# boycehbz/MvSMPLfitting

Measured on AMD Instinct MI355X. Metric: L-BFGS closure evaluations per second (fwd+bwd, all concurrently fitted problems), 8-view 1-person 4-stage fits, higher is better.
Workload: dtype f32

## Files before the change

### mvsmplfitting_amd/csrc/closure_device.h

```cpp
#pragma once
#include <cstddef>
#include "mvfit_device.h"

namespace mvfit {

struct ObsBlock {
    float camR[MVFIT_MAX_VIEWS][9];
    float camt[MVFIT_MAX_VIEWS][3];
    float camf[MVFIT_MAX_VIEWS];
    float camc[MVFIT_MAX_VIEWS][2];
    float gt[MVFIT_MAX_VIEWS * NKP * 2];
    float wc[MVFIT_MAX_VIEWS * NKP];
    float gt3d[NKP * 3];
    float c3d[NKP];
};
struct PoseBlock {
    float theta[72];
    float R[NJ][9];
    float rod[NJ][3];
    float J[NJ][3];
    float Mj[32][12];
    float G[NJ][12];
    float A[NJ][12];
};
// ... 492 lines not shown
            L.pose.Mj[j][4 * (e / 3) + (e % 3)] = (j == 0 ? L.opt.x[X_SC] : 1.0f) * sel;
            if (e < 3) L.pose.rod[j][e] = rod[e];
        } else {
            const int a = e - 9;
            const int pa = L.M.parents[j];
            float s = L.M.J_t[3 * j + a];
#pragma unroll
            for (int l = 0; l < 10; ++l) s = fmaf(L.M.J_S[3 * j + a][l], L.opt.x[X_BETAS + l], s);
            float sp = 0.f;
            if (j > 0) {
                sp = L.M.J_t[3 * pa + a];
#pragma unroll
                for (int l = 0; l < 10; ++l) sp = fmaf(L.M.J_S[3 * pa + a][l], L.opt.x[X_BETAS + l], sp);
            }
            L.pose.J[j][a] = s;
            L.pose.Mj[j][4 * a + 3] = s - sp;
        }
    }
    __syncthreads();
}

template <bool REMOTE = false>
__device__ __attribute__((noinline)) void pose_prep_decode(const DevModel& M, ClosureLds& L, uint32_t flags, int tid) {
    pose_prep_decode_inl<REMOTE>(M, L, flags, tid);
}

template <bool CALL = false>
__device__ __forceinline__ void pose_prep(const DevModel& M, ClosureLds& L, uint32_t flags, int tid) {
    if constexpr (CALL) pose_prep_decode<false>(M, L, flags, tid);
    else pose_prep_decode_inl<false>(M, L, flags, tid);
    pose_prep_elems(M, L, flags, tid);
}

__device__ __forceinline__ void chain_forward_wave(ClosureLds& L, int lane) {
    if (lane < 12) L.pose.G[0][lane] = L.pose.Mj[0][lane];
    const int q = lane / 12, e = lane - 12 * q, a = e >> 2, c = e & 3;
    const int npass = L.M.n_fwd;
    constexpr int CH = 8;
    wave_lds_fence();
    for (int p0 = 0; p0 < npass; p0 += CH) {
        int w[CH];
        float m0[CH], m1[CH], m2[CH];
#pragma unroll
        for (int u = 0; u < CH; ++u) w[u] = (q < 5 && p0 + u < npass) ? L.M.fwd_tab[p0 + u][q] : -1;
#pragma unroll
        for (int u = 0; u < CH; ++u) {
            const int j = w[u] >= 0 ? (w[u] & 0xff) : 0;
            m0[u] = L.pose.Mj[j][c]; m1[u] = L.pose.Mj[j][4 + c]; m2[u] = L.pose.Mj[j][8 + c];
        }
#pragma unroll
        for (int u = 0; u < CH; ++u) {
            if (p0 + u < npass) {
                if (w[u] >= 0) {
                    const int j = w[u] & 0xff, pa = w[u] >> 8;
                    const float4 g = *reinterpret_cast<const float4*>(&L.pose.G[pa][4 * a]);
                    float v = g.x * m0[u] + g.y * m1[u] + g.z * m2[u];
                    if (c == 3) v += g.w;
                    L.pose.G[j][e] = v;
                }
                wave_lds_fence();
            }
        }
    }
    for (int i = lane; i < NJ * 3; i += 64) {
        const int j = i / 3, aa = i - 3 * j;
        const float4 g = *reinterpret_cast<const float4*>(&L.pose.G[j][4 * aa]);
        const float t = g.w - (g.x * L.pose.J[j][0] + g.y * L.pose.J[j][1] + g.z * L.pose.J[j][2]);
        *reinterpret_cast<float4*>(&L.pose.A[j][4 * aa]) = make_float4(g.x, g.y, g.z, t);
    }
}

__device__ __forceinline__ void chain_forward_block(ClosureLds& L, int tid) {
    const bool act = tid < NJ * 12;
    const int j = act ? tid / 12 : 0, e = tid - 12 * j, a = e >> 2, c = e & 3;
    const int ns = L.M.n_jump;
    int anc[5];
#pragma unroll
    for (int s = 0; s < 5; ++s) anc[s] = L.M.anc_tab[s][j];
    const float* src = &L.pose.Mj[0][0];
    float* dst = &L.pose.G[0][0];
#pragma unroll
    for (int s = 0; s < 5; ++s) {
        if (s < ns) {
            if (act) {
                float v;
                if (anc[s] >= 0) {
                    const float4 x = *reinterpret_cast<const float4*>(src + anc[s] * 12 + 4 * a);
                    v = x.x * src[j * 12 + c] + x.y * src[j * 12 + 4 + c] + x.z * src[j * 12 + 8 + c];
                    if (c == 3) v += x.w;
                } else {
                    v = src[j * 12 + e];
                }
                dst[j * 12 + e] = v;
            }
            __syncthreads();
            src = dst;
// ... 303 lines not shown
            const float* mu = M.gmm_means + m * 69;
            float qd = 0.f;
            for (int r = l16; r < 69; r += 16) qd = fmaf(L.gmm_t[m][r], L.pose.theta[3 + r] - mu[r], qd);
            qd = row16_sum(qd);
            if (l16 == 0) L.gmm_ll[m] = 0.5f * qd - M.gmm_lognw[m];
        }
    }
    __syncthreads();
    double total = 0.0;
    if constexpr (!DEFER) total = loss_combine<false>(M, L, V, W, tid == 0);
    const bool use_3d = (W.flags & MVFIT_F_USE_3D) != 0;
    if (want_grad && tid < 3) {
        float s = 0.f;
        for (int w = 0; w < ndw; ++w) s += L.red_f[w][tid];
        if (use_3d) for (int k = 0; k < NKP; ++k) s += L.gkp3[k][tid];
        L.gtau[tid] = s;
    }
    if (want_grad && tid >= 64 && tid < 64 + NKP * 3) {
        const int i = tid - 64;
        float s = 0.f;
#pragma unroll
        for (int vv = 0; vv < MVFIT_MAX_VIEWS; ++vv) if (vv < V) s += (&L.gkp_part[vv][0][0])[i];
        if (use_3d) s += (&L.gkp3[0][0])[i];
        (&L.gkp[0][0])[i] = s;
    }
    return total;
}

__device__ __forceinline__ void chain_backward_wave(ClosureLds& L, int lane) {
    const int q = lane / 12, e = lane - 12 * q, a = e >> 2, m = e & 3;
    const int mr = m < 3 ? m : 0;
    const int npass = L.M.n_bwd;
    constexpr int CH = 4;
    wave_lds_fence();
    for (int p0 = 0; p0 < npass; p0 += CH) {
        int w[CH];
        float4 k0[CH], k1[CH], k2[CH];
        float own[CH];
#pragma unroll
        for (int u = 0; u < CH; ++u) w[u] = (q < 5 && p0 + u < npass) ? L.M.bwd_tab[p0 + u][q] : -1;
#pragma unroll
        for (int u = 0; u < CH; ++u) {
            const int ww = w[u] != -1 ? w[u] : 0x1f1f1f00;
            const int c0 = (ww >> 8) & 0xff, c1 = (ww >> 16) & 0xff, c2 = (ww >> 24) & 0xff;
            k0[u] = *reinterpret_cast<const float4*>(&L.pose.Mj[c0][4 * mr]);
            k1[u] = *reinterpret_cast<const float4*>(&L.pose.Mj[c1][4 * mr]);
            k2[u] = *reinterpret_cast<const float4*>(&L.pose.Mj[c2][4 * mr]);
            own[u] = L.gG[ww & 0x1f][e];
        }
#pragma unroll
        for (int u = 0; u < CH; ++u) {
            if (p0 + u < npass) {
                if (w[u] != -1) {
                    const int p = w[u] & 0x1f, c0 = (w[u] >> 8) & 0xff, c1 = (w[u] >> 16) & 0xff, c2 = (w[u] >> 24) & 0xff;
                    const float4 g0 = *reinterpret_cast<const float4*>(&L.gG[c0][4 * a]);
                    const float4 g1 = *reinterpret_cast<const float4*>(&L.gG[c1][4 * a]);
                    const float4 g2 = *reinterpret_cast<const float4*>(&L.gG[c2][4 * a]);
                    float acc;
                    if (m < 3) {
                        acc = (g0.x * k0[u].x + g0.y * k0[u].y + g0.z * k0[u].z + g0.w * k0[u].w) +
                              (g1.x * k1[u].x + g1.y * k1[u].y + g1.z * k1[u].z + g1.w * k1[u].w) +
                              (g2.x * k2[u].x + g2.y * k2[u].y + g2.z * k2[u].z + g2.w * k2[u].w);
                    } else {
                        acc = g0.w + g1.w + g2.w;
                    }
                    const float base = (w[u] & 0x80) ? L.gG[p][e] : own[u];
                    L.gG[p][e] = base + acc;
                }
                wave_lds_fence();
            }
        }
    }
}

constexpr int BWD_SLICES = 8, BWD_CPS = NC_MAX / BWD_SLICES;
__device__ __forceinline__ int bwd_slices(int) { return BWD_SLICES; }

template <int CPS>
__device__ __forceinline__ void contraction_backward_t(const DevModel& M, ClosureLds& L, int t, int nthreads) {
    constexpr int npq = KROWS >> 2;
    const int nc_pad = L.M.nc_pad;
    const int cps = ((nc_pad >> 2) + BWD_SLICES - 1) / BWD_SLICES * 4;
    for (int item = t; item < npq * BWD_SLICES; item += nthreads) {
        const int pq = item % npq, cs = (item / npq + (int)blockIdx.x) & (BWD_SLICES - 1);
        const int c0 = cs * cps;
        const float4* src = reinterpret_cast<const float4*>(M.pd_subT) + pq;
        float4 v[CPS];
#pragma unroll
        for (int r = 0; r < CPS; ++r) {
            const int c = min(c0 + r, nc_pad - 1);
            if (CPS == BWD_CPS ? r < cps : true) v[r] = src[(size_t)c * npq];
        }
        float4 acc0 = make_float4(0.f, 0.f, 0.f, 0.f), acc1 = acc0;
#pragma unroll
        for (int r = 0; r < CPS; r += 2) {
            if (r < cps) {
                const float g0 = L.gvp[c0 + r], g1 = L.gvp[c0 + r + 1];
                acc0.x = fmaf(g0, v[r].x, acc0.x); acc0.y = fmaf(g0, v[r].y, acc0.y);
                acc0.z = fmaf(g0, v[r].z, acc0.z); acc0.w = fmaf(g0, v[r].w, acc0.w);
                acc1.x = fmaf(g1, v[r + 1].x, acc1.x); acc1.y = fmaf(g1, v[r + 1].y, acc1.y);
                acc1.z = fmaf(g1, v[r + 1].z, acc1.z); acc1.w = fmaf(g1, v[r + 1].w, acc1.w);
            }
        }
        float4* dst = reinterpret_cast<float4*>(L.scratch + cs * KROWS + 4 * pq);
        *dst = make_float4(acc0.x + acc1.x, acc0.y + acc1.y, acc0.z + acc1.z, acc0.w + acc1.w);
    }
}

__device__ __forceinline__ void contraction_backward(const DevModel& M, ClosureLds& L, int t, int nthreads) {
    constexpr int SMPL_CPS = 28;
    if (((L.M.nc_pad >> 2) + BWD_SLICES - 1) / BWD_SLICES * 4 <= SMPL_CPS) contraction_backward_t<SMPL_CPS>(M, L, t, nthreads);
    else contraction_backward_t<BWD_CPS>(M, L, t, nthreads);
}

template <bool REMOTE = false, bool DEFER = false, bool SDFW = false>
__device__ __forceinline__ void closure_backward(const DevModel& M, ClosureLds& L, int V, const DevWeights& W, int tid) {
    const bool use_vp = (W.flags & MVFIT_F_VPOSER) != 0;
    const int ns = L.M.ns, nc = L.M.nc, nc_pad = L.M.nc_pad;
    __syncthreads();
    if constexpr (DEFER) {
        static_assert(NC_MAX + NJ * 3 <= STEP_NT - 64, "E5's threads leave the last wave free");
        if (tid >= STEP_NT - 64) loss_combine<SDFW>(M, L, V, W, tid == STEP_NT - 64);
    }
    if (tid < nc_pad) {
        float v = 0.f;
        if (tid < nc) {
            const int s = tid / 3, bq = tid - 3 * s;
            float gx0 = 0.f, gx1 = 0.f, gx2 = 0.f;
            if (L.M.padded) {
#pragma unroll
                for (int t = 0; t < VS_NZ; ++t) {
                    const int k = L.M.vsp_k[s][t];
                    const float w = L.M.vsp_w[s][t];
                    gx0 = fmaf(w, L.gkp[k][0], gx0); gx1 = fmaf(w, L.gkp[k][1], gx1); gx2 = fmaf(w, L.gkp[k][2], gx2);
                }
            } else {
                for (int t = L.M.vs_start[s]; t < L.M.vs_start[s + 1]; ++t) {
                    const int k = L.M.vs_k[t];
                    const float w = L.M.vs_w[t];
                    gx0 = fmaf(w, L.gkp[k][0], gx0); gx1 = fmaf(w, L.gkp[k][1], gx1); gx2 = fmaf(w, L.gkp[k][2], gx2);
                }
            }
            v = L.T[s][0 + bq] * gx0 + L.T[s][4 + bq] * gx1 + L.T[s][8 + bq] * gx2;
            L.gx[tid] = bq == 0 ? gx0 : (bq == 1 ? gx1 : gx2);
        }
        L.gvp[tid] = v;
    } else if (tid < NC_MAX) {
        L.gvp[tid] = 0.f;
    } else if (tid < NC_MAX + NJ * 3 && L.M.n_skel) {
        const int i = tid - NC_MAX, j = i / 3, a = i - 3 * j;
        float gs = 0.f;
        for (int k = 0; k < NKP; ++k) if (kp_joint_of(L.M, k) == j) gs += L.gkp[k][a];
        L.gM[j][a] = gs;
    }
    __syncthreads();
    PH_T(4);
    const float sdf_fac = L.sdf_fac;
    if (tid < NJ * 16) {
        const int j = tid >> 4, g = tid & 15;
        float acc[12];
#pragma unroll
        for (int e = 0; e < 12; ++e) acc[e] = 0.f;
        for (int s = g; s < ns; s += 16) {
            const float w = L.M.wT[j][s];
            const float g0 = w * L.gx[3 * s], g1 = w * L.gx[3 * s + 1], g2 = w * L.gx[3 * s + 2];
            const float v0 = L.vposed[3 * s], v1 = L.vposed[3 * s + 1], v2 = L.vposed[3 * s + 2];
            acc[0] = fmaf(g0, v0, acc[0]); acc[1] = fmaf(g0, v1, acc[1]); acc[2] = fmaf(g0, v2, acc[2]);
            acc[3] = fmaf(g1, v0, acc[3]); acc[4] = fmaf(g1, v1, acc[4]); acc[5] = fmaf(g1, v2, acc[5]);
            acc[6] = fmaf(g2, v0, acc[6]); acc[7] = fmaf(g2, v1, acc[7]); acc[8] = fmaf(g2, v2, acc[8]);
            acc[9] += g0; acc[10] += g1; acc[11] += g2;
        }
#pragma unroll
        for (int e = 0; e < 12; ++e) acc[e] = row16_sum(acc[e]);
        if (g == 0) {
            if (sdf_fac != 0.f) {
#pragma unroll
                for (int e = 0; e < 12; ++e) acc[e] = fmaf(sdf_fac, sdf_ld(&L.sdf_adj->gA[j * 12 + e]), acc[e]);
            }
            const float J0 = L.pose.J[j][0], J1 = L.pose.J[j][1], J2 = L.pose.J[j][2];
#pragma unroll
            for (int a = 0; a < 3; ++a) {
                *reinterpret_cast<float4*>(&L.gG[j][4 * a]) =
                    make_float4(acc[3 * a + 0] - acc[9 + a] * J0, acc[3 * a + 1] - acc[9 + a] * J1,
                                acc[3 * a + 2] - acc[9 + a] * J2, L.M.n_skel ? acc[9 + a] + L.gM[j][a] : acc[9 + a]);
                L.gJ[j][a] = -(L.pose.G[j][0 + a] * acc[9] + L.pose.G[j][4 + a] * acc[10] + L.pose.G[j][8 + a] * acc[11]);
            }
        }
    }
    __syncthreads();
    PH_T(5);
    const long long t_e7 = PH_CLK();
    if (tid < 64) { chain_backward_wave(L, tid); PH_T(23); }
    else { contraction_backward(M, L, tid - 64, STEP_NT - 64); PH_W(59, 64, t_e7); PH_W(61, 448, t_e7); }
    const int ncs = bwd_slices(STEP_NT - 64);
    __syncthreads();
    PH_T(6);
    auto gm_elem = [&](int pa, int j, int mm, int c) -> float {
        float v = L.pose.G[pa][mm] * L.gG[j][c] + L.pose.G[pa][4 + mm] * L.gG[j][4 + c] + L.pose.G[pa][8 + mm] * L.gG[j][8 + c];
        asm volatile("" : "+v"(v));
        return v;
    };
    constexpr int GJ_T0 = 320;
    static_assert(GJ_T0 >= NJ * 12 && GJ_T0 % 64 == 0 && GJ_T0 + NJ * 3 <= STEP_NT, "g_J totals on otherwise idle waves");
    if (tid >= GJ_T0 && tid < GJ_T0 + NJ * 3) {
        const int i = tid - GJ_T0, j = i / 3, a = i - 3 * j;
        const int c_lo = L.M.child_start[j], c_hi = L.M.child_start[j + 1];
        int ch[3];
#pragma unroll
        for (int k = 0; k < 3; ++k) ch[k] = c_lo + k < c_hi ? L.M.child_list[min(c_lo + k, NJ - 1)] : NJ;
        float gj = L.gJ[j][a] + (j == 0 ? L.gG[0][4 * a + 3] : gm_elem(L.M.parents[j], j, a, 3));
        float sub[3];
#pragma unroll
        for (int k = 0; k < 3; ++k) sub[k] = gm_elem(j, ch[k], a, 3);
#pragma unroll
        for (int k = 0; k < 3; ++k) gj -= sub[k];
        for (int ci = c_lo + 3; ci < c_hi; ++ci) gj -= gm_elem(j, L.M.child_list[ci], a, 3);
        L.gvp[i] = gj;
    }
    if (tid < NJ * 12) {
        const int j = tid / 12, e = tid - 12 * j, mm = e >> 2, c = e & 3;
        float v;
        if (j == 0) v = L.gG[0][e];
        else {
            const int pa = L.M.parents[j];
            v = L.pose.G[pa][mm] * L.gG[j][c] + L.pose.G[pa][4 + mm] * L.gG[j][4 + c] + L.pose.G[pa][8 + mm] * L.gG[j][8 + c];
        }
        L.gM[j][e] = v;
// ... 228 lines not shown
```

### mvsmplfitting_amd/csrc/model_layout.h

```cpp
#pragma once
#include <stdint.h>

namespace mvfit {

constexpr int NJ = 24;
constexpr int NKP = 17;
constexpr int KROWS = 224;
constexpr int KGROUPS = 28;
constexpr int TILE_V = 32;
constexpr int NS_MAX = 96;
constexpr int NS_STRIDE = 112;
constexpr int NC_MAX = NS_MAX * 3;
constexpr int KNNZ_MAX = 160;
constexpr int KP_NZ = 12;
constexpr int VS_NZ = 2;
constexpr int VPS_SLICES = 8;

struct ModelLds {
    float wT[NJ][NS_STRIDE];
    float J_t[NJ * 3];
    float J_S[NJ * 3][11];
    float vt_sub[NC_MAX];
    int sel_v[NS_MAX];
    int kp_start[NKP + 1];
    int kp_s[KNNZ_MAX];
    float kp_w[KNNZ_MAX];
    int vs_start[NS_MAX + 1];
    int vs_k[KNNZ_MAX];
    float vs_w[KNNZ_MAX];
    int kpp_s[NKP][KP_NZ];
    float kpp_w[NKP][KP_NZ];
    int vsp_k[NS_MAX][VS_NZ];
    float vsp_w[NS_MAX][VS_NZ];
    int padded;
    unsigned kp_joint[3];
    int parents[NJ];
    int nlevels;
    int level_start[NJ + 1];
    int level_joints[NJ];
    int child_start[NJ + 1];
    int child_list[NJ];
    int n_fwd, n_bwd;
    int fwd_tab[NJ][5];
    int bwd_tab[NJ][5];
    int anc_tab[5][NJ];
    int n_jump, n_skel, jpad1, jpad2;
    int ns, nc, nc_pad, pad0;
    float selw[NS_MAX][4];
    unsigned selj[NS_MAX];
    int sel_sparse, spad0, spad1, spad2;
};
static_assert(sizeof(ModelLds) % 16 == 0, "ModelLds is bulk-copied as 16-byte words");
static_assert(NKP <= 18 && NJ < 31, "kp_joint packs six 5-bit entries per word");

}
```

### mvsmplfitting_amd/csrc/model_prep.cpp

```cpp
#include "model_prep.h"

#include <math.h>
#include <algorithm>
#include <cmath>
#include <cstdarg>
#include <cstdio>
#include <cstring>

namespace mvfit {
namespace {

constexpr int NPOSE = 207;
constexpr int NBASIS = 217;

int fail(std::string& err, int code, const char* fmt, ...) {
    char buf[512];
    va_list ap;
    va_start(ap, fmt);
    vsnprintf(buf, sizeof(buf), fmt, ap);
    va_end(ap);
    err = buf;
    return code;
}

// ... 165 lines not shown
    for (int s = 0; s < ns; ++s) {
        G.vs_start[s] = nnz;
        for (int k = 0; k < NKP; ++k) {
            const double w = ksel[(size_t)k * nv + sel[s]];
            if (w == 0.0) continue;
            G.vs_k[nnz] = k; G.vs_w[nnz] = (float)w; ++nnz;
        }
    }
    for (int s = ns; s <= NS_MAX; ++s) G.vs_start[s] = nnz;
    G.padded = 1;
    for (int k = 0; k < NKP; ++k) {
        const int n0 = G.kp_start[k], cnt = G.kp_start[k + 1] - n0;
        if (cnt > KP_NZ) G.padded = 0;
        for (int t = 0; t < KP_NZ; ++t) { G.kpp_s[k][t] = t < cnt ? G.kp_s[n0 + t] : 0; G.kpp_w[k][t] = t < cnt ? G.kp_w[n0 + t] : 0.f; }
    }
    for (int s = 0; s < NS_MAX; ++s) {
        const int n0 = G.vs_start[s], cnt = G.vs_start[s + 1] - n0;
        if (cnt > VS_NZ) G.padded = 0;
        for (int t = 0; t < VS_NZ; ++t) { G.vsp_k[s][t] = t < cnt ? G.vs_k[n0 + t] : 0; G.vsp_w[s][t] = t < cnt ? G.vs_w[n0 + t] : 0.f; }
    }
    h.tile_sel_start.assign(h.ntiles + 1, 0);
    h.tile_sel_local.assign(ns, 0);
    h.tile_sel_slot.assign(ns, 0);
    int pos = 0;
    for (int T = 0; T < h.ntiles; ++T) {
        h.tile_sel_start[T] = pos;
        for (int s = 0; s < ns; ++s)
            if (sel[s] / TILE_V == T) { h.tile_sel_local[pos] = sel[s] % TILE_V; h.tile_sel_slot[pos] = s; ++pos; }
    }
    h.tile_sel_start[h.ntiles] = pos;
    return MVFIT_OK;
}

int build_chain(const mvfit_model& m, ModelLds& G, std::string& err) {
    int depth[NJ];
    for (int j = 0; j < NJ; ++j) {
        G.parents[j] = m.parents[j];
        if (j > 0 && (m.parents[j] < 0 || m.parents[j] >= j)) return fail(err, MVFIT_E_ARG, "parents must be topologically ordered");
        depth[j] = j == 0 ? 0 : depth[m.parents[j]] + 1;
    }
    int maxd = 0;
    for (int j = 0; j < NJ; ++j) maxd = std::max(maxd, depth[j]);
    G.nlevels = maxd + 1;
    int pos = 0;
    for (int lv = 0; lv <= maxd; ++lv) {
        G.level_start[lv] = pos;
        for (int j = 0; j < NJ; ++j) if (depth[j] == lv) G.level_joints[pos++] = j;
    }
    for (int lv = maxd + 1; lv <= NJ; ++lv) G.level_start[lv] = pos;
    pos = 0;
    for (int p = 0; p < NJ; ++p) {
        G.child_start[p] = pos;
        for (int j = 1; j < NJ; ++j) if (m.parents[j] == p) G.child_list[pos++] = j;
    }
    G.child_start[NJ] = pos;
    memset(G.fwd_tab, 0xff, sizeof(G.fwd_tab));
    memset(G.bwd_tab, 0xff, sizeof(G.bwd_tab));
    int np = 0;
    for (int lv = 1; lv <= maxd; ++lv)
        for (int base = G.level_start[lv]; base < G.level_start[lv + 1]; base += 5, ++np) {
            if (np >= NJ) return fail(err, MVFIT_E_UNSUPPORTED, "kinematic tree needs more than %d chain passes", NJ);
            for (int q = 0; q < 5 && base + q < G.level_start[lv + 1]; ++q) {
                const int j = G.level_joints[base + q];
                G.fwd_tab[np][q] = j | (m.parents[j] << 8);
            }
        }
// ... 11 lines not shown
    np = 0;
    for (int lv = maxd - 1; lv >= 0; --lv) {
        std::vector<int> entries;
        for (int i = G.level_start[lv]; i < G.level_start[lv + 1]; ++i) {
            const int p = G.level_joints[i];
            const int nc = G.child_start[p + 1] - G.child_start[p];
            for (int k = 0; k < nc; k += 3) {
                int ch[3] = {31, 31, 31};
                for (int t = 0; t < 3 && k + t < nc; ++t) ch[t] = G.child_list[G.child_start[p] + k + t];
                entries.push_back(p | (k > 0 ? 0x80 : 0) | (ch[0] << 8) | (ch[1] << 16) | (ch[2] << 24));
            }
        }
        std::vector<bool> used(entries.size(), false);
        size_t left = entries.size();
        while (left > 0) {
            if (np >= NJ) return fail(err, MVFIT_E_UNSUPPORTED, "kinematic tree needs more than %d adjoint passes", NJ);
            int q = 0;
            std::vector<int> parents_in_pass;
            for (size_t i = 0; i < entries.size() && q < 5; ++i) {
                if (used[i]) continue;
                const int p = entries[i] & 0x1f;
                bool clash = false;
                for (int pp : parents_in_pass) clash |= pp == p;
                if (clash) continue;
                G.bwd_tab[np][q++] = entries[i];
                parents_in_pass.push_back(p);
                used[i] = true;
                --left;
            }
            ++np;
        }
    }
    G.n_bwd = np;
    return MVFIT_OK;
}

int build_vposer(const mvfit_model& m, HostModel& h, std::string& err) {
    if (!m.vp_fc1_w) return MVFIT_OK;
    if (!m.vp_fc1_b || !m.vp_fc2_w || !m.vp_fc2_b || !m.vp_out_w || !m.vp_out_b) return fail(err, MVFIT_E_ARG, "incomplete vposer weights");
    const std::vector<float>&w1 = h.vp_w1, &w2 = h.vp_w2, &w3 = h.vp_w3;
    h.vp_w1.assign(m.vp_fc1_w, m.vp_fc1_w + 512 * 32); h.vp_b1.assign(m.vp_fc1_b, m.vp_fc1_b + 512);
    h.vp_w2.assign(m.vp_fc2_w, m.vp_fc2_w + 512 * 512); h.vp_b2.assign(m.vp_fc2_b, m.vp_fc2_b + 512);
    h.vp_w3.assign(m.vp_out_w, m.vp_out_w + 138 * 512); h.vp_b3.assign(m.vp_out_b, m.vp_out_b + 138);
    h.vp_w1T.assign(32 * 512, 0.f); h.vp_w2T.assign(512 * 512, 0.f); h.vp_w3T.assign(512 * 144, 0.f);
    for (int o = 0; o < 512; ++o) for (int i = 0; i < 32; ++i) h.vp_w1T[i * 512 + o] = w1[o * 32 + i];
    for (int o = 0; o < 512; ++o) for (int i = 0; i < 512; ++i) h.vp_w2T[i * 512 + o] = w2[o * 512 + i];
    for (int o = 0; o < 138; ++o) for (int i = 0; i < 512; ++i) h.vp_w3T[i * 144 + o] = w3[o * 512 + i];
    h.vp_tw2.assign((size_t)VPS_SLICES * 16 * 512 * 4, 0.f);
    h.vp_tw3.assign((size_t)VPS_SLICES * 6 * 512 * 4, 0.f);
    for (int hs = 0; hs < VPS_SLICES; ++hs)
        for (int tid = 0; tid < 512; ++tid) {
            const int w = tid >> 6, l = tid & 63;
            for (int j = 0; j < 16; ++j)
                for (int q = 0; q < 4; ++q)
                    h.vp_tw2[(((size_t)hs * 16 + j) * 512 + tid) * 4 + q] = w2[(size_t)(64 * hs + 8 * w + (j >> 1)) * 512 + 8 * l + 4 * (j & 1) + q];
            for (int j = 0; j < 6; ++j) {
                const int o = l + 64 * (j >> 1);
                if (o < 138)
                    for (int q = 0; q < 4; ++q)
                        h.vp_tw3[(((size_t)hs * 6 + j) * 512 + tid) * 4 + q] = w3[(size_t)o * 512 + 64 * hs + 8 * w + 4 * (j & 1) + q];
            }
        }
    h.has_vposer = true;
    return MVFIT_OK;
}

// ... 58 lines not shown
```

### mvsmplfitting_amd/csrc/mvfit_api.hip

```cpp
#include <dlfcn.h>
#include <hip/hip_runtime.h>

#include <algorithm>
#include <cmath>
#include <cstdarg>
#include <cstdio>
#include <cstdlib>
#include <cstring>
#include <string>
#include <vector>

#include "closure_device.h"
#include "model_prep.h"

namespace mvfit {

hipError_t launch_vertex_pass(const DevModel& M, const DevPose& P, int B, float* verts, int ksplit,
                              hipStream_t stream, hipEvent_t ev_start = nullptr, hipEvent_t ev_stop = nullptr);
hipError_t vertex_pass_configure();
hipError_t launch_pass_gate(const DevPose& P, int b_lo, int B, hipStream_t stream);
hipError_t launch_vertex_pass_resident(const DevModel& M, const ResidentArgs& RA, int tpw, hipStream_t stream);
hipError_t launch_sdf_term(const DevModel& M, const DevPose& P, const float* verts, int B, const int32_t* faces, int num_faces,
                           int G, const int* gate, SdfBox* box, float4* samp, void* entries, SdfAdj* adj, hipStream_t stream,
                           void* cull, unsigned* answer_tag = nullptr, unsigned answer = 0u, const unsigned long long* box_parts = nullptr);
// ... 261 lines not shown
        for (int e = 0; e < LB_EPL; ++e) {
            const int i = LB_EPL * tid + e;
            gnew[e] = i < D ? L.grad[cmap(i, use_vp)] : 0.f;
        }
    }
    lbfgs_round<float, STEP_NT, REUSE>(&L.opt.lbS, &L.opt.lbV[0], H, L.lbW, O, (double)(float)total, gnew, xt, tid, stage_final, [&]() {
        PH_T(10);
        if constexpr (COMPACT) lb_direction_compact<float, STEP_NT>(H, L.lbW, tid);
        else lb_direction_block<float, STEP_NT>(H, L.lbW, tid, GL);
        PH_T(11); PH_ADD(15, 1);
    });
    if (tid < 64) {
#pragma unroll
        for (int e = 0; e < LB_EPL; ++e) {
            const int i = LB_EPL * tid + e;
            if (i < D) L.opt.x[cmap(i, use_vp)] = xt[e];
        }
        if (tid == 0) { L.sh_stage = min(L.opt.lbS.stage, O.num_stages - 1); L.sh_status = L.opt.lbS.status; }
        PH_ADD(13, 1); PH_ADD(14, L.opt.lbS.hist_len);
    }
    __syncthreads();
    PH_T(12);
    return L.sh_status != 0;
}

constexpr int kHistLdFull = 88, kHistLdVp = 52;
__host__ __device__ constexpr int persistent_hist_ld(bool vp) { return vp ? kHistLdVp : kHistLdFull; }
__host__ __device__ constexpr size_t persistent_tail_offset(bool vp) {
    return vp ? ((sizeof(ClosureLds) + 15) & ~(size_t)15) : offsetof(ClosureLds, vp_pre1);
}
__host__ __device__ constexpr size_t persistent_lds_bytes(bool vp) {
    return persistent_tail_offset(vp) + ((size_t)2 * LB_HIST * persistent_hist_ld(vp) + LB_RPACK) * sizeof(float);
}
static_assert(persistent_lds_bytes(false) <= 160 * 1024 && persistent_lds_bytes(true) <= 160 * 1024, "one workgroup per CU: 160 KB of LDS");

__device__ __forceinline__ size_t step_lds_dev() { return (sizeof(ClosureLds) + 15) & ~(size_t)15; }

template <bool REUSE>
__global__ __launch_bounds__(STEP_NT) void fit_step_kernel(DevModel M, const ObsBlock* __restrict__ obs, int nviews,
                                                           StageWeights SW, LbOpts O, DevPose P, FitBuffers F) {
    extern __shared__ __attribute__((aligned(16))) unsigned char smem_raw[];
    ClosureLds& L = *reinterpret_cast<ClosureLds*>(smem_raw);
    const int b = blockIdx.x, tid = threadIdx.x;
    PH_T0();
    prologue(L, M, obs + b, F.pose + b, F.opt + b, P.vposed_sel + (size_t)b * NC_MAX, P.xs_sel + (size_t)b * NC_MAX, nullptr, tid,
             F.sdf_adj ? F.sdf_adj + b : nullptr, (SW.w[0].flags & MVFIT_F_VPOSER) ? F.vp + b : nullptr);
    opts_in(L, SW, O, tid);
    __syncthreads();
    if (L.opt.lbS.status != 0) return;
    if (tid == 0) { L.sh_stage = L.opt.lbS.stage; L.sh_status = 0; }
    LbHist<float> H{F.dirs + (size_t)b * LB_HIST * LB_D, F.stps + (size_t)b * LB_HIST * LB_D, L.opt.lb_ro,
                    F.grow + (size_t)b * LB_GSIZE, F.gcol + (size_t)b * LB_GSIZE};
    __syncthreads();
    float warm = 0.f;
    {
        const int n0 = L.opt.lbS.hist_len, head0 = L.opt.lbS.hist_head;
        constexpr int LPR = LB_D * 4 / 128;
        if (tid < 2 * LPR * n0) {
            const int which = tid / (LPR * n0), r = tid - which * LPR * n0, age = r / LPR, ln = r - age * LPR;
            int slot = head0 + age;
            slot = slot >= LB_HIST ? slot - LB_HIST : slot;
            warm = (which ? H.stps : H.dirs)[slot * LB_D + ln * 32];
        }
    }
    LbGramLds GL{reinterpret_cast<float*>(smem_raw + step_lds_dev()), L.opt.lbS.hist_head,
                 min(L.opt.lbS.hist_len + 1, LB_HIST) + 3 + 4 * LB_PD};
    lb_gram_dma<STEP_NT>(H.gcol, GL.row0, GL.buf, GL.nrows, tid);
// ... 1823 lines not shown
```

Baseline: 1.544 million.

## Pass kinematic chain values through lane shuffles and rebalance backward contraction across waves

```diff
diff --git a/mvsmplfitting_amd/csrc/closure_device.h b/mvsmplfitting_amd/csrc/closure_device.h
--- a/mvsmplfitting_amd/csrc/closure_device.h
+++ b/mvsmplfitting_amd/csrc/closure_device.h
@@ -548,17 +548,48 @@
     pose_prep_elems(M, L, flags, tid);
 }
 
+template <int SEL>
+__device__ __forceinline__ float quad_bcast(float v) { return dpp_mov<SEL * 0x55>(v); }
+__device__ __forceinline__ float lane_fetch(float v, int src_lane) {
+    return __builtin_bit_cast(float, __builtin_amdgcn_ds_bpermute(src_lane << 2, __builtin_bit_cast(int, v)));
+}
+__device__ __forceinline__ float4 quad_row(float t) {
+    return make_float4(quad_bcast<0>(t), quad_bcast<1>(t), quad_bcast<2>(t), quad_bcast<3>(t));
+}
+
+__device__ __forceinline__ float chain_fwd_elem(const float4& g, float m0, float m1, float m2, bool last_col) {
+#pragma clang fp contract(off)
+    const float p1 = g.y * m1, p2 = g.z * m2;
+    float v = fmaf(g.x, m0, p1) + p2;
+    if (last_col) v += g.w;
+    return v;
+}
+__device__ __forceinline__ float chain_bwd_elem(const float4& g0, const float4& g1, const float4& g2, const float4& k0,
+                                                const float4& k1, const float4& k2, bool rot) {
+#pragma clang fp contract(off)
+    if (!rot) return g0.w + g1.w + g2.w;
+    const float a0 = ((g0.x * k0.x + g0.y * k0.y) + g0.z * k0.z) + g0.w * k0.w;
+    const float a1 = fmaf(g1.w, k1.w, fmaf(g1.z, k1.z, fmaf(g1.y, k1.y, g1.x * k1.x)));
+    const float a2 = fmaf(g2.w, k2.w, fmaf(g2.z, k2.z, fmaf(g2.y, k2.y, g2.x * k2.x)));
+    return (a0 + a1) + a2;
+}
+
 __device__ __forceinline__ void chain_forward_wave(ClosureLds& L, int lane) {
-    if (lane < 12) L.pose.G[0][lane] = L.pose.Mj[0][lane];
     const int q = lane / 12, e = lane - 12 * q, a = e >> 2, c = e & 3;
+    float cur = lane < 12 ? L.pose.Mj[0][lane] : 0.f;
+    if (lane < 12) L.pose.G[0][lane] = cur;
     const int npass = L.M.n_fwd;
     constexpr int CH = 8;
-    wave_lds_fence();
     for (int p0 = 0; p0 < npass; p0 += CH) {
-        int w[CH];
+        int w[CH], src[CH], fb[CH];
         float m0[CH], m1[CH], m2[CH];
 #pragma unroll
-        for (int u = 0; u < CH; ++u) w[u] = (q < 5 && p0 + u < npass) ? L.M.fwd_tab[p0 + u][q] : -1;
+        for (int u = 0; u < CH; ++u) {
+            const bool in = q < 5 && p0 + u < npass;
+            w[u] = in ? L.M.fwd_tab[p0 + u][q] : -1;
+            src[u] = in ? (int)L.M.fwd_src[p0 + u][q] : 0xff;
+            fb[u] = p0 + u < npass ? (int)L.M.fwd_src[p0 + u][5] : 0;
+        }
 #pragma unroll
         for (int u = 0; u < CH; ++u) {
             const int j = w[u] >= 0 ? (w[u] & 0xff) : 0;
@@ -567,17 +598,20 @@
 #pragma unroll
         for (int u = 0; u < CH; ++u) {
             if (p0 + u < npass) {
+                float4 g = quad_row(lane_fetch(cur, 12 * (src[u] & 7) + e));
+                const bool lds = wave_uniform(fb[u]) != 0;
+                if (lds) wave_lds_fence();
                 if (w[u] >= 0) {
                     const int j = w[u] & 0xff, pa = w[u] >> 8;
-                    const float4 g = *reinterpret_cast<const float4*>(&L.pose.G[pa][4 * a]);
-                    float v = g.x * m0[u] + g.y * m1[u] + g.z * m2[u];
-                    if (c == 3) v += g.w;
+                    if (lds && src[u] == 0xff) g = *reinterpret_cast<const float4*>(&L.pose.G[pa][4 * a]);
+                    const float v = chain_fwd_elem(g, m0[u], m1[u], m2[u], c == 3);
                     L.pose.G[j][e] = v;
+                    cur = v;
                 }
-                wave_lds_fence();
-            }
-        }
-    }
+            }
+        }
+    }
+    wave_lds_fence();
     for (int i = lane; i < NJ * 3; i += 64) {
         const int j = i / 3, aa = i - 3 * j;
         const float4 g = *reinterpret_cast<const float4*>(&L.pose.G[j][4 * aa]);
@@ -947,13 +981,19 @@
     const int mr = m < 3 ? m : 0;
     const int npass = L.M.n_bwd;
     constexpr int CH = 4;
+    float cur = 0.f;
     wave_lds_fence();
     for (int p0 = 0; p0 < npass; p0 += CH) {
-        int w[CH];
-        float4 k0[CH], k1[CH], k2[CH];
+        int w[CH], src[CH], fb[CH];
+        float4 k0[CH], k1[CH], k2[CH], s0[CH], s1[CH], s2[CH];
         float own[CH];
 #pragma unroll
-        for (int u = 0; u < CH; ++u) w[u] = (q < 5 && p0 + u < npass) ? L.M.bwd_tab[p0 + u][q] : -1;
+        for (int u = 0; u < CH; ++u) {
+            const bool in = q < 5 && p0 + u < npass;
+            w[u] = in ? L.M.bwd_tab[p0 + u][q] : -1;
+            src[u] = in ? (int)L.M.bwd_src[p0 + u][q] : 0;
+            fb[u] = p0 + u < npass ? (int)L.M.fwd_src[p0 + u][6] : 0;
+        }
 #pragma unroll
         for (int u = 0; u < CH; ++u) {
             const int ww = w[u] != -1 ? w[u] : 0x1f1f1f00;
@@ -962,152 +1002,202 @@
             k1[u] = *reinterpret_cast<const float4*>(&L.pose.Mj[c1][4 * mr]);
             k2[u] = *reinterpret_cast<const float4*>(&L.pose.Mj[c2][4 * mr]);
             own[u] = L.gG[ww & 0x1f][e];
+            s0[u] = *reinterpret_cast<const float4*>(&L.gG[c0][4 * a]);
+            s1[u] = *reinterpret_cast<const float4*>(&L.gG[c1][4 * a]);
+            s2[u] = *reinterpret_cast<const float4*>(&L.gG[c2][4 * a]);
         }
 #pragma unroll
         for (int u = 0; u < CH; ++u) {
             if (p0 + u < npass) {
+                const int b0 = src[u] & 0xf, b1 = (src[u] >> 4) & 0xf, b2 = (src[u] >> 8) & 0xf;
+                const float4 f0 = quad_row(lane_fetch(cur, 12 * (b0 & 7) + e));
+                const float4 f1 = quad_row(lane_fetch(cur, 12 * (b1 & 7) + e));
+                const float4 f2 = quad_row(lane_fetch(cur, 12 * (b2 & 7) + e));
+                const bool lds = wave_uniform(fb[u]) != 0;
+                if (lds) wave_lds_fence();
                 if (w[u] != -1) {
                     const int p = w[u] & 0x1f, c0 = (w[u] >> 8) & 0xff, c1 = (w[u] >> 16) & 0xff, c2 = (w[u] >> 24) & 0xff;
-                    const float4 g0 = *reinterpret_cast<const float4*>(&L.gG[c0][4 * a]);
-                    const float4 g1 = *reinterpret_cast<const float4*>(&L.gG[c1][4 * a]);
-                    const float4 g2 = *reinterpret_cast<const float4*>(&L.gG[c2][4 * a]);
-                    float acc;
-                    if (m < 3) {
-                        acc = (g0.x * k0[u].x + g0.y * k0[u].y + g0.z * k0[u].z + g0.w * k0[u].w) +
-                              (g1.x * k1[u].x + g1.y * k1[u].y + g1.z * k1[u].z + g1.w * k1[u].w) +
-                              (g2.x * k2[u].x + g2.y * k2[u].y + g2.z * k2[u].z + g2.w * k2[u].w);
-                    } else {
-                        acc = g0.w + g1.w + g2.w;
+                    float4 g0 = b0 == 0xe ? s0[u] : f0;
+                    float4 g1 = b1 == 0xe ? s1[u] : f1;
+                    float4 g2 = b2 == 0xe ? s2[u] : f2;
+                    const bool on_lds = lds && (src[u] & 0x1000) != 0;
+                    if (on_lds) {
+                        g0 = *reinterpret_cast<const float4*>(&L.gG[c0][4 * a]);
+                        g1 = *reinterpret_cast<const float4*>(&L.gG[c1][4 * a]);
+                        g2 = *reinterpret_cast<const float4*>(&L.gG[c2][4 * a]);
                     }
-                    const float base = (w[u] & 0x80) ? L.gG[p][e] : own[u];
-                    L.gG[p][e] = base + acc;
+                    const float acc = chain_bwd_elem(g0, g1, g2, k0[u], k1[u], k2[u], m < 3);
+                    const float base = (on_lds && (w[u] & 0x80)) ? L.gG[p][e] : own[u];
+                    const float r = base + acc;
+                    L.gG[p][e] = r;
+                    cur = r;
                 }
-                wave_lds_fence();
-            }
-        }
-    }
+            }
+        }
+    }
+    wave_lds_fence();
 }
 
 constexpr int BWD_SLICES = 8, BWD_CPS = NC_MAX / BWD_SLICES;
 __device__ __forceinline__ int bwd_slices(int) { return BWD_SLICES; }
 
+constexpr int BWD_ITEMS = (KROWS >> 2) * BWD_SLICES;
+__device__ __forceinline__ int bwd_cps(const ClosureLds& L) { return ((L.M.nc_pad >> 2) + BWD_SLICES - 1) / BWD_SLICES * 4; }
+
 template <int CPS>
-__device__ __forceinline__ void contraction_backward_t(const DevModel& M, ClosureLds& L, int t, int nthreads) {
+__device__ __forceinline__ void bwd_item_load(const DevModel& M, const ClosureLds& L, int item, float4 (&v)[CPS]) {
     constexpr int npq = KROWS >> 2;
     const int nc_pad = L.M.nc_pad;
-    const int cps = ((nc_pad >> 2) + BWD_SLICES - 1) / BWD_SLICES * 4;
-    for (int item = t; item < npq * BWD_SLICES; item += nthreads) {
-        const int pq = item % npq, cs = (item / npq + (int)blockIdx.x) & (BWD_SLICES - 1);
-        const int c0 = cs * cps;
-        const float4* src = reinterpret_cast<const float4*>(M.pd_subT) + pq;
+    const int cps = bwd_cps(L);
+    const int pq = item % npq, cs = (item / npq + (int)blockIdx.x) & (BWD_SLICES - 1);
+    const int c0 = cs * cps;
+    const float4* src = reinterpret_cast<const float4*>(M.pd_subT) + pq;
+#pragma unroll
+    for (int r = 0; r < CPS; ++r) {
+        const int c = min(c0 + r, nc_pad - 1);
+        if (CPS == BWD_CPS ? r < cps : true) v[r] = src[(size_t)c * npq];
+    }
+}
+
+template <int CPS>
+__device__ __forceinline__ void bwd_item_sum(ClosureLds& L, int item, const float4 (&v)[CPS]) {
+    constexpr int npq = KROWS >> 2;
+    const int cps = bwd_cps(L);
+    const int pq = item % npq, cs = (item / npq + (int)blockIdx.x) & (BWD_SLICES - 1);
+    const int c0 = cs * cps;
+    float4 acc0 = make_float4(0.f, 0.f, 0.f, 0.f), acc1 = acc0;
+#pragma unroll
+    for (int r = 0; r < CPS; r += 2) {
+        if (r < cps) {
+            const float g0 = L.gvp[c0 + r], g1 = L.gvp[c0 + r + 1];
+            acc0.x = fmaf(g0, v[r].x, acc0.x); acc0.y = fmaf(g0, v[r].y, acc0.y);
+            acc0.z = fmaf(g0, v[r].z, acc0.z); acc0.w = fmaf(g0, v[r].w, acc0.w);
+            acc1.x = fmaf(g1, v[r + 1].x, acc1.x); acc1.y = fmaf(g1, v[r + 1].y, acc1.y);
+            acc1.z = fmaf(g1, v[r + 1].z, acc1.z); acc1.w = fmaf(g1, v[r + 1].w, acc1.w);
+        }
+    }
+    float4* dst = reinterpret_cast<float4*>(L.scratch + cs * KROWS + 4 * pq);
+    *dst = make_float4(acc0.x + acc1.x, acc0.y + acc1.y, acc0.z + acc1.z, acc0.w + acc1.w);
+}
+
+constexpr int SMPL_CPS = 28;
+template <int CPS>
+__device__ __forceinline__ void bwd_stream_batches(const DevModel& M, ClosureLds& L, int sb, int sb_end, bool streamw, int tid) {
+    bool at_e5 = streamw;
+    long long t_s = PH_CLK();
+    for (; sb < sb_end; ++sb) {
         float4 v[CPS];
-#pragma unroll
-        for (int r = 0; r < CPS; ++r) {
-            const int c = min(c0 + r, nc_pad - 1);
-            if (CPS == BWD_CPS ? r < cps : true) v[r] = src[(size_t)c * npq];
-        }
-        float4 acc0 = make_float4(0.f, 0.f, 0.f, 0.f), acc1 = acc0;
-#pragma unroll
-        for (int r = 0; r < CPS; r += 2) {
-            if (r < cps) {
-                const float g0 = L.gvp[c0 + r], g1 = L.gvp[c0 + r + 1];
-                acc0.x = fmaf(g0, v[r].x, acc0.x); acc0.y = fmaf(g0, v[r].y, acc0.y);
-                acc0.z = fmaf(g0, v[r].z, acc0.z); acc0.w = fmaf(g0, v[r].w, acc0.w);
-                acc1.x = fmaf(g1, v[r + 1].x, acc1.x); acc1.y = fmaf(g1, v[r + 1].y, acc1.y);
-                acc1.z = fmaf(g1, v[r + 1].z, acc1.z); acc1.w = fmaf(g1, v[r + 1].w, acc1.w);
-            }
-        }
-        float4* dst = reinterpret_cast<float4*>(L.scratch + cs * KROWS + 4 * pq);
-        *dst = make_float4(acc0.x + acc1.x, acc0.y + acc1.y, acc0.z + acc1.z, acc0.w + acc1.w);
-    }
-}
-
-__device__ __forceinline__ void contraction_backward(const DevModel& M, ClosureLds& L, int t, int nthreads) {
-    constexpr int SMPL_CPS = 28;
-    if (((L.M.nc_pad >> 2) + BWD_SLICES - 1) / BWD_SLICES * 4 <= SMPL_CPS) contraction_backward_t<SMPL_CPS>(M, L, t, nthreads);
-    else contraction_backward_t<BWD_CPS>(M, L, t, nthreads);
-}
+        bwd_item_load<CPS>(M, L, 64 * sb + (tid & 63), v);
+        if (at_e5) { __syncthreads(); at_e5 = false; t_s = PH_CLK(); }
+        bwd_item_sum<CPS>(L, 64 * sb + (tid & 63), v);
+    }
+    if (tid >= 64) { PH_W(59, 64, t_s); PH_W(61, 448, t_s); }
+    if (streamw) {
+        if (at_e5) __syncthreads();
+        __syncthreads();
+    }
+}
+
+#ifndef MVFIT_BWD_EARLY6
+#define MVFIT_BWD_EARLY6 2
+#endif
+#ifndef MVFIT_BWD_EARLY7
+#define MVFIT_BWD_EARLY7 1
+#endif
+constexpr int BWD_EARLY6 = MVFIT_BWD_EARLY6, BWD_EARLY7 = MVFIT_BWD_EARLY7, BWD_BATCHES = BWD_ITEMS / 64;
+static_assert(BWD_ITEMS % 64 == 0 && BWD_EARLY6 >= 1 && BWD_EARLY7 >= 0 && BWD_BATCHES - BWD_EARLY6 - BWD_EARLY7 <= 5 &&
+              BWD_EARLY6 + BWD_EARLY7 <= BWD_BATCHES, "the rest of the transposed stream is one batch per wave of waves 1-5");
 
 template <bool REMOTE = false, bool DEFER = false, bool SDFW = false>
 __device__ __forceinline__ void closure_backward(const DevModel& M, ClosureLds& L, int V, const DevWeights& W, int tid) {
     const bool use_vp = (W.flags & MVFIT_F_VPOSER) != 0;
     const int ns = L.M.ns, nc = L.M.nc, nc_pad = L.M.nc_pad;
     __syncthreads();
-    if constexpr (DEFER) {
-        static_assert(NC_MAX + NJ * 3 <= STEP_NT - 64, "E5's threads leave the last wave free");
-        if (tid >= STEP_NT - 64) loss_combine<SDFW>(M, L, V, W, tid == STEP_NT - 64);
-    }
-    if (tid < nc_pad) {
-        float v = 0.f;
-        if (tid < nc) {
-            const int s = tid / 3, bq = tid - 3 * s;
-            float gx0 = 0.f, gx1 = 0.f, gx2 = 0.f;
-            if (L.M.padded) {
-#pragma unroll
-                for (int t = 0; t < VS_NZ; ++t) {
-                    const int k = L.M.vsp_k[s][t];
-                    const float w = L.M.vsp_w[s][t];
-                    gx0 = fmaf(w, L.gkp[k][0], gx0); gx1 = fmaf(w, L.gkp[k][1], gx1); gx2 = fmaf(w, L.gkp[k][2], gx2);
+    static_assert(NC_MAX + NJ * 3 <= STEP_NT - 128 && NJ * 16 <= STEP_NT - 128, "E5's and E6's threads leave the last two waves free");
+    const int wv = wave_uniform(tid >> 6);
+    const bool streamw = wv >= STEP_NW - 2;
+    int sb = 0, sb_end = 0;
+    if (streamw) {
+        if constexpr (DEFER) {
+            if (wv == STEP_NW - 1) loss_combine<SDFW>(M, L, V, W, tid == STEP_NT - 64);
+        }
+        sb = wv == STEP_NW - 2 ? 0 : BWD_EARLY6;
+        sb_end = wv == STEP_NW - 2 ? BWD_EARLY6 : BWD_EARLY6 + BWD_EARLY7;
+    } else {
+        if (tid < nc_pad) {
+            float v = 0.f;
+            if (tid < nc) {
+                const int s = tid / 3, bq = tid - 3 * s;
+                float gx0 = 0.f, gx1 = 0.f, gx2 = 0.f;
+                if (L.M.padded) {
+#pragma unroll
+                    for (int t = 0; t < VS_NZ; ++t) {
+                        const int k = L.M.vsp_k[s][t];
+                        const float w = L.M.vsp_w[s][t];
+                        gx0 = fmaf(w, L.gkp[k][0], gx0); gx1 = fmaf(w, L.gkp[k][1], gx1); gx2 = fmaf(w, L.gkp[k][2], gx2);
+                    }
+                } else {
+                    for (int t = L.M.vs_start[s]; t < L.M.vs_start[s + 1]; ++t) {
+                        const int k = L.M.vs_k[t];
+                        const float w = L.M.vs_w[t];
+                        gx0 = fmaf(w, L.gkp[k][0], gx0); gx1 = fmaf(w, L.gkp[k][1], gx1); gx2 = fmaf(w, L.gkp[k][2], gx2);
+                    }
                 }
-            } else {
-                for (int t = L.M.vs_start[s]; t < L.M.vs_start[s + 1]; ++t) {
-                    const int k = L.M.vs_k[t];
-                    const float w = L.M.vs_w[t];
-                    gx0 = fmaf(w, L.gkp[k][0], gx0); gx1 = fmaf(w, L.gkp[k][1], gx1); gx2 = fmaf(w, L.gkp[k][2], gx2);
+                v = L.T[s][0 + bq] * gx0 + L.T[s][4 + bq] * gx1 + L.T[s][8 + bq] * gx2;
+                L.gx[tid] = bq == 0 ? gx0 : (bq == 1 ? gx1 : gx2);
+            }
+            L.gvp[tid] = v;
+        } else if (tid < NC_MAX) {
+            L.gvp[tid] = 0.f;
+        } else if (tid < NC_MAX + NJ * 3 && L.M.n_skel) {
+            const int i = tid - NC_MAX, j = i / 3, a = i - 3 * j;
+            float gs = 0.f;
+            for (int k = 0; k < NKP; ++k) if (kp_joint_of(L.M, k) == j) gs += L.gkp[k][a];
+            L.gM[j][a] = gs;
+        }
+        __syncthreads();
+        PH_T(4);
+        const float sdf_fac = L.sdf_fac;
+        if (tid < NJ * 16) {
+            const int j = tid >> 4, g = tid & 15;
+            float acc[12];
+#pragma unroll
+            for (int e = 0; e < 12; ++e) acc[e] = 0.f;
+            for (int s = g; s < ns; s += 16) {
+                const float w = L.M.wT[j][s];
+                const float g0 = w * L.gx[3 * s], g1 = w * L.gx[3 * s + 1], g2 = w * L.gx[3 * s + 2];
+                const float v0 = L.vposed[3 * s], v1 = L.vposed[3 * s + 1], v2 = L.vposed[3 * s + 2];
+                acc[0] = fmaf(g0, v0, acc[0]); acc[1] = fmaf(g0, v1, acc[1]); acc[2] = fmaf(g0, v2, acc[2]);
+                acc[3] = fmaf(g1, v0, acc[3]); acc[4] = fmaf(g1, v1, acc[4]); acc[5] = fmaf(g1, v2, acc[5]);
+                acc[6] = fmaf(g2, v0, acc[6]); acc[7] = fmaf(g2, v1, acc[7]); acc[8] = fmaf(g2, v2, acc[8]);
+                acc[9] += g0; acc[10] += g1; acc[11] += g2;
+            }
+#pragma unroll
+            for (int e = 0; e < 12; ++e) acc[e] = row16_sum(acc[e]);
+            if (g == 0) {
+                if (sdf_fac != 0.f) {
+#pragma unroll
+                    for (int e = 0; e < 12; ++e) acc[e] = fmaf(sdf_fac, sdf_ld(&L.sdf_adj->gA[j * 12 + e]), acc[e]);
                 }
-            }
-            v = L.T[s][0 + bq] * gx0 + L.T[s][4 + bq] * gx1 + L.T[s][8 + bq] * gx2;
-            L.gx[tid] = bq == 0 ? gx0 : (bq == 1 ? gx1 : gx2);
-        }
-        L.gvp[tid] = v;
-    } else if (tid < NC_MAX) {
-        L.gvp[tid] = 0.f;
-    } else if (tid < NC_MAX + NJ * 3 && L.M.n_skel) {
-        const int i = tid - NC_MAX, j = i / 3, a = i - 3 * j;
-        float gs = 0.f;
-        for (int k = 0; k < NKP; ++k) if (kp_joint_of(L.M, k) == j) gs += L.gkp[k][a];
-        L.gM[j][a] = gs;
-    }
-    __syncthreads();
-    PH_T(4);
+                const float J0 = L.pose.J[j][0], J1 = L.pose.J[j][1], J2 = L.pose.J[j][2];
+#pragma unroll
+                for (int a = 0; a < 3; ++a) {
+                    *reinterpret_cast<float4*>(&L.gG[j][4 * a]) =
+                        make_float4(acc[3 * a + 0] - acc[9 + a] * J0, acc[3 * a + 1] - acc[9 + a] * J1,
+                                    acc[3 * a + 2] - acc[9 + a] * J2, L.M.n_skel ? acc[9 + a] + L.gM[j][a] : acc[9 + a]);
+                    L.gJ[j][a] = -(L.pose.G[j][0 + a] * acc[9] + L.pose.G[j][4 + a] * acc[10] + L.pose.G[j][8 + a] * acc[11]);
+                }
+            }
+        }
+        __syncthreads();
+        PH_T(5);
+        if (wv == 0) { chain_backward_wave(L, tid); PH_T(23); }
+        else if (wv <= BWD_BATCHES - BWD_EARLY6 - BWD_EARLY7) { sb = BWD_EARLY6 + BWD_EARLY7 + wv - 1; sb_end = sb + 1; }
+    }
+    if (wave_uniform(bwd_cps(L)) <= SMPL_CPS) bwd_stream_batches<SMPL_CPS>(M, L, sb, sb_end, streamw, tid);
+    else bwd_stream_batches<BWD_CPS>(M, L, sb, sb_end, streamw, tid);
+    const int ncs = bwd_slices(STEP_NT - 64);
     const float sdf_fac = L.sdf_fac;
-    if (tid < NJ * 16) {
-        const int j = tid >> 4, g = tid & 15;
-        float acc[12];
-#pragma unroll
-        for (int e = 0; e < 12; ++e) acc[e] = 0.f;
-        for (int s = g; s < ns; s += 16) {
-            const float w = L.M.wT[j][s];
-            const float g0 = w * L.gx[3 * s], g1 = w * L.gx[3 * s + 1], g2 = w * L.gx[3 * s + 2];
-            const float v0 = L.vposed[3 * s], v1 = L.vposed[3 * s + 1], v2 = L.vposed[3 * s + 2];
-            acc[0] = fmaf(g0, v0, acc[0]); acc[1] = fmaf(g0, v1, acc[1]); acc[2] = fmaf(g0, v2, acc[2]);
-            acc[3] = fmaf(g1, v0, acc[3]); acc[4] = fmaf(g1, v1, acc[4]); acc[5] = fmaf(g1, v2, acc[5]);
-            acc[6] = fmaf(g2, v0, acc[6]); acc[7] = fmaf(g2, v1, acc[7]); acc[8] = fmaf(g2, v2, acc[8]);
-            acc[9] += g0; acc[10] += g1; acc[11] += g2;
-        }
-#pragma unroll
-        for (int e = 0; e < 12; ++e) acc[e] = row16_sum(acc[e]);
-        if (g == 0) {
-            if (sdf_fac != 0.f) {
-#pragma unroll
-                for (int e = 0; e < 12; ++e) acc[e] = fmaf(sdf_fac, sdf_ld(&L.sdf_adj->gA[j * 12 + e]), acc[e]);
-            }
-            const float J0 = L.pose.J[j][0], J1 = L.pose.J[j][1], J2 = L.pose.J[j][2];
-#pragma unroll
-            for (int a = 0; a < 3; ++a) {
-                *reinterpret_cast<float4*>(&L.gG[j][4 * a]) =
-                    make_float4(acc[3 * a + 0] - acc[9 + a] * J0, acc[3 * a + 1] - acc[9 + a] * J1,
-                                acc[3 * a + 2] - acc[9 + a] * J2, L.M.n_skel ? acc[9 + a] + L.gM[j][a] : acc[9 + a]);
-                L.gJ[j][a] = -(L.pose.G[j][0 + a] * acc[9] + L.pose.G[j][4 + a] * acc[10] + L.pose.G[j][8 + a] * acc[11]);
-            }
-        }
-    }
-    __syncthreads();
-    PH_T(5);
-    const long long t_e7 = PH_CLK();
-    if (tid < 64) { chain_backward_wave(L, tid); PH_T(23); }
-    else { contraction_backward(M, L, tid - 64, STEP_NT - 64); PH_W(59, 64, t_e7); PH_W(61, 448, t_e7); }
-    const int ncs = bwd_slices(STEP_NT - 64);
     __syncthreads();
     PH_T(6);
     auto gm_elem = [&](int pa, int j, int mm, int c) -> float {
diff --git a/mvsmplfitting_amd/csrc/model_layout.h b/mvsmplfitting_amd/csrc/model_layout.h
--- a/mvsmplfitting_amd/csrc/model_layout.h
+++ b/mvsmplfitting_amd/csrc/model_layout.h
@@ -43,6 +43,8 @@
     int n_fwd, n_bwd;
     int fwd_tab[NJ][5];
     int bwd_tab[NJ][5];
+    unsigned char fwd_src[NJ][8];
+    unsigned short bwd_src[NJ][5];
     int anc_tab[5][NJ];
     int n_jump, n_skel, jpad1, jpad2;
     int ns, nc, nc_pad, pad0;
diff --git a/mvsmplfitting_amd/csrc/model_prep.cpp b/mvsmplfitting_amd/csrc/model_prep.cpp
--- a/mvsmplfitting_amd/csrc/model_prep.cpp
+++ b/mvsmplfitting_amd/csrc/model_prep.cpp
@@ -221,6 +221,43 @@
     return MVFIT_OK;
 }
 
+static void build_chain_sources(ModelLds& G) {
+    memset(G.fwd_src, 0, sizeof(G.fwd_src));
+    memset(G.bwd_src, 0, sizeof(G.bwd_src));
+    int pass_of[NJ], slot_of[NJ];
+    pass_of[0] = -1; slot_of[0] = 0;
+    for (int ps = 0; ps < G.n_fwd; ++ps)
+        for (int q = 0; q < 5; ++q) {
+            G.fwd_src[ps][q] = 0xff;
+            if (G.fwd_tab[ps][q] < 0) continue;
+            const int j = G.fwd_tab[ps][q] & 0xff, pa = G.fwd_tab[ps][q] >> 8;
+            pass_of[j] = ps; slot_of[j] = q;
+            if (pass_of[pa] == ps - 1) G.fwd_src[ps][q] = (unsigned char)slot_of[pa];
+            else G.fwd_src[ps][5] = 1;
+        }
+    int last_pass[32], last_slot[32];
+    for (int j = 0; j < 32; ++j) last_pass[j] = last_slot[j] = -1;
+    for (int ps = 0; ps < G.n_bwd; ++ps)
+        for (int q = 0; q < 5; ++q)
+            if (G.bwd_tab[ps][q] != -1) { last_pass[G.bwd_tab[ps][q] & 0x1f] = ps; last_slot[G.bwd_tab[ps][q] & 0x1f] = q; }
+    for (int ps = 0; ps < G.n_bwd; ++ps)
+        for (int q = 0; q < 5; ++q) {
+            const int w = G.bwd_tab[ps][q];
+            if (w == -1) continue;
+            bool lds = (w & 0x80) != 0;
+            unsigned word = 0;
+            for (int k = 0; k < 3; ++k) {
+                const int c = (w >> (8 + 8 * k)) & 0xff;
+                unsigned s = 0xe;
+                if (c < NJ && last_pass[c] >= 0) s = last_pass[c] == ps - 1 ? (unsigned)last_slot[c] : 0xfu;
+                lds |= s == 0xf;
+                word |= s << (4 * k);
+            }
+            G.bwd_src[ps][q] = (unsigned short)(word | (lds ? 0x1000u : 0u));
+            if (lds) G.fwd_src[ps][6] = 1;
+        }
+}
+
 int build_chain(const mvfit_model& m, ModelLds& G, std::string& err) {
     int depth[NJ];
     for (int j = 0; j < NJ; ++j) {
@@ -298,6 +335,7 @@
         }
     }
     G.n_bwd = np;
+    build_chain_sources(G);
     return MVFIT_OK;
 }
 
diff --git a/mvsmplfitting_amd/csrc/mvfit_api.hip b/mvsmplfitting_amd/csrc/mvfit_api.hip
--- a/mvsmplfitting_amd/csrc/mvfit_api.hip
+++ b/mvsmplfitting_amd/csrc/mvfit_api.hip
@@ -317,7 +317,9 @@
 __host__ __device__ constexpr size_t persistent_lds_bytes(bool vp) {
     return persistent_tail_offset(vp) + ((size_t)2 * LB_HIST * persistent_hist_ld(vp) + LB_RPACK) * sizeof(float);
 }
-static_assert(persistent_lds_bytes(false) <= 160 * 1024 && persistent_lds_bytes(true) <= 160 * 1024, "one workgroup per CU: 160 KB of LDS");
+constexpr size_t kStaticLdsReserve = 256;
+static_assert(persistent_lds_bytes(false) + kStaticLdsReserve <= 160 * 1024 && persistent_lds_bytes(true) + kStaticLdsReserve <= 160 * 1024,
+              "one workgroup per CU: 160 KB of LDS");
 
 __device__ __forceinline__ size_t step_lds_dev() { return (sizeof(ClosureLds) + 15) & ~(size_t)15; }
 
```

Result: slower. 1.127 million (-27.0%).
